# sen-ye/dmvae

Measured on AMD Instinct MI355X. Metric: images/sec DMVAE train step @256x256, higher is better.
Workload: dtype bf16

## Files before the change

### dmvae_amd/csrc/gemm_pp.hip

```cpp
#include "common.h"
#include "dmvae_hip.h"
#include <cstdlib>
#include <type_traits>

constexpr int GEMM_MAXBUF = 6;

namespace dmvae_gemm_pp {

struct Args {
  const bf16* x;
  const bf16* w;
  const void* bias;
  void* y;
  int M, N, K, lda, ldw, ldy;
  int act, bias_bf16;
  int H;
  unsigned wbytes;
  unsigned wsRow, wsK;
  int ntn, total;
  float inv_ntn;
  int tpb;
  float inv_tpb;
  unsigned sA, sB, sY, xbytes, ybytes;
  unsigned long long* dbg;
  int V, skS, T;
  float* slabs;
  unsigned* counters;
  unsigned slab_bytes;
  void* y2;
  int ldy2;
};

constexpr int SK_COHERENT = 1 | 16;
constexpr unsigned SENT = 0x80000000u;

__device__ __forceinline__ int swz64(int row) { return (0 - (row >> 2)) & 3; }

template <int N>
__device__ __forceinline__ void wait_vmcnt() {
  __builtin_amdgcn_s_waitcnt((N & 15) | 0x0F70 | ((N >> 4) << 14));
  asm volatile("" ::: "memory");
}

__device__ __forceinline__ float gelu_f(float x) { return dmvae_gelu_f(x); }

template <int TM, int TP, int WM, int WP, bool OUT_F32, int NBUF, bool BATCHED = false, bool SK = false>
__global__ __launch_bounds__(WM * WP * 64) void gemm_pp_kernel(Args a) {
#if __HIP_DEVICE_COMPILE__
  constexpr int PF = NBUF - 1;
  static_assert(!(SK && BATCHED) && !(SK && OUT_F32), "SK: single product, bf16 result");
  constexpr int CL = TM / WM / 16, BT = TP / WP / 16;
  constexpr int NW = WM * WP;
  static_assert(NW == 8 && CL * 16 * WM == TM && BT * 16 * WP == TP && CL * BT <= 32 && (CL == 4 || CL == 6 || CL == 8), "wave grid");
  constexpr int TILE_A = TM * 64, TILE_B = TP * 64, SLOT = TILE_A + TILE_B, RING = NBUF * SLOT;
  constexpr int NPA = (TM / 16 + NW - 1) / NW, NPB = (TP / 16 + NW - 1) / NW, NP = NPA + NPB;
  constexpr int CW = CL * 16;
  constexpr int BIAS_OFF = RING, DUMP_OFF = RING + 2048;
  constexpr int SPR = OUT_F32 ? (CL + 3) / 4 : 1;
  constexpr int NST = BT * 4 * SPR;
  extern __shared__ __attribute__((aligned(16))) char smem[];
  typedef unsigned u32x4 __attribute__((ext_vector_type(4)));
  typedef unsigned u32x3 __attribute__((ext_vector_type(3)));
  typedef unsigned u32x2 __attribute__((ext_vector_type(2)));

  const int tid = threadIdx.x, lane = tid & 63;
  const int wave = __builtin_amdgcn_readfirstlane(tid >> 6);
  const int grp = wave >> 2;
  const int wm = wave / WP, wp = wave % WP;
  const int nK = a.K >> 5;
  const unsigned bsz = a.bias_bf16 ? 2u : 4u;
  const bool gated = a.act == 6;
  const float inv_ntn = a.inv_ntn;

  const __amdgpu_buffer_rsrc_t rA = __builtin_amdgcn_make_buffer_rsrc((void*)a.w, 0, a.wbytes, 0x00020000);
  const __amdgpu_buffer_rsrc_t rB = __builtin_amdgcn_make_buffer_rsrc((void*)a.x, 0, BATCHED ? a.xbytes : (unsigned)a.M * (unsigned)a.lda * 2u, 0x00020000);
  const __amdgpu_buffer_rsrc_t rBias = __builtin_amdgcn_make_buffer_rsrc((void*)a.bias, 0, a.bias ? (unsigned)a.N * bsz : 0u, 0x00020000);
  const __amdgpu_buffer_rsrc_t rY = __builtin_amdgcn_make_buffer_rsrc(a.y, 0, BATCHED ? a.ybytes : (unsigned)a.M * (unsigned)a.ldy * (OUT_F32 ? 4u : 2u), 0x00020000);
  const __amdgpu_buffer_rsrc_t rY2 = __builtin_amdgcn_make_buffer_rsrc(a.y2, 0, a.y2 ? (unsigned)a.M * (unsigned)a.ldy2 * 2u : 0u, 0x00020000);

  auto calc = [&](unsigned work, unsigned (&vA)[NPA], unsigned (&vB)[NPB], unsigned& vBias, int& m0, int& n0, int& b0) {
    int lane_c = lane;
    asm volatile("" : "+v"(lane_c));
    const bool live = work < (unsigned)a.total;
    int wid = live ? (SK ? (int)work : (int)xcd_remap(work, a.total)) : 0;
    unsigned offA = 0, offB = 0;
    b0 = 0;
    if constexpr (BATCHED) {
      int b = (int)((float)wid * a.inv_tpb);
      int r = wid - b * a.tpb;
      if (r < 0) { b--; r += a.tpb; }
      if (r >= a.tpb) { b++; r -= a.tpb; }
      b0 = __builtin_amdgcn_readfirstlane(b);
      wid = r;
      offA = (unsigned)b0 * a.sA; offB = (unsigned)b0 * a.sB;
    }
    int mt = (int)((float)wid * inv_ntn);
    int nt = wid - mt * a.ntn;
    if (nt < 0) { mt--; nt += a.ntn; }
    if (nt >= a.ntn) { mt++; nt -= a.ntn; }
    m0 = __builtin_amdgcn_readfirstlane(mt) * TP;
    n0 = __builtin_amdgcn_readfirstlane(nt) * TM;
#pragma unroll
    for (int p = 0; p < NPA; p++) {
      const int rl = (wave * NPA + p) * 16 + (lane_c >> 2);
      const int wmr = rl / CW, r = rl % CW, i = r >> 4, c = r & 15;
      int n = n0 + wmr * CW + CL * c + i;
      bool n_ok = n < a.N;
      if (gated) {
        const int hid = (n0 >> 1) + wmr * (CW / 2) + (CL / 2) * c + (i % (CL / 2));
        n = (i < CL / 2 ? 0 : a.H) + hid;
        n_ok = hid < a.H;
      }
      const int ch = (lane_c & 3) ^ swz64(rl);
      vA[p] = (live && rl < TM && n_ok) ? (unsigned)n * a.wsRow + ch * 16u + offA : SENT;
    }
#pragma unroll
    for (int p = 0; p < NPB; p++) {
      const int rl = (wave * NPB + p) * 16 + (lane_c >> 2);
      const int m = m0 + rl;
      const int ch = (lane_c & 3) ^ swz64(rl);
      vB[p] = (live && rl < TP && m < a.M) ? (unsigned)m * (unsigned)a.lda * 2u + ch * 16u + offB : SENT;
    }
    const unsigned e0 = (unsigned)lane_c * (16u / bsz);
    if (gated) {
      const unsigned eh = e0 < (unsigned)(TM / 2) ? e0 : e0 - (unsigned)(TM / 2);
      const unsigned hid = (unsigned)(n0 >> 1) + eh;
      vBias = (live && wave == 0 && e0 < (unsigned)TM && hid < (unsigned)a.H) ? ((e0 < (unsigned)(TM / 2) ? 0u : (unsigned)a.H) + hid) * bsz : SENT;
    } else {
      vBias = (live && wave == 0 && e0 < (unsigned)TM && (unsigned)n0 + e0 < (unsigned)a.N) ? ((unsigned)n0 + e0) * bsz : SENT;
    }
  };
  auto issue_k = [&](const unsigned (&vA)[NPA], const unsigned (&vB)[NPB], unsigned kt, int slot) {
#pragma unroll
    for (int p = 0; p < NPA; p++) {
      const int g = wave * NPA + p;
      __builtin_amdgcn_raw_ptr_buffer_load_lds(rA, LPTR(smem + (g * 16 < TM ? slot + g * 1024 : DUMP_OFF)), 16, vA[p], kt * a.wsK, 0, 0);
    }
#pragma unroll
    for (int p = 0; p < NPB; p++) {
      const int g = wave * NPB + p;
      __builtin_amdgcn_raw_ptr_buffer_load_lds(rB, LPTR(smem + (g * 16 < TP ? slot + TILE_A + g * 1024 : DUMP_OFF)), 16, vB[p], kt * 64u, 0, 0);
    }
  };
  auto issue_bias = [&](unsigned vBias, int par) {
    __builtin_amdgcn_raw_ptr_buffer_load_lds(rBias, LPTR(smem + (wave == 0 ? BIAS_OFF + par * 1024 : DUMP_OFF)), 16, vBias, 0, 0, 0);
  };

  const int fr = (lane & 15) * 64 + (((lane >> 4) ^ swz64(lane & 15)) << 4);
  const int wbase = wm * (CW * 64) + fr;
  const int tbase = TILE_A + wp * (TP / WP) * 64 + fr;

  constexpr int MINSEG = 2 * PF + 2;
  struct Unit { int tile, kb, nk, p, P, i1; };
  auto bnd = [&](int v) -> int {
    if (a.skS > 0) {
      const int t = v / a.skS, p = v - t * a.skS;
      return t * nK + (p * nK) / a.skS;
    }
    int b = (int)((long long)v * (long long)a.T / (long long)a.V);
    const int r = b % nK;
    if (r < MINSEG) b -= r;
    else if (nK - r < MINSEG) b += nK - r;
    return b;
  };
  unsigned sk_work = blockIdx.x;
  int sk_pos = 0, sk_end = 0, sk_v = 0;
  bool sk_started = false;
  auto next_unit = [&]() -> Unit {
    Unit u = {a.total, 0, 2 * PF, 0, 1, 0};
    while (sk_pos >= sk_end) {
      if (sk_started) sk_work += gridDim.x;
      sk_started = true;
      if (sk_work >= (unsigned)a.V) return u;
      sk_v = (int)xcd_remap(sk_work, (unsigned)a.V);
      sk_pos = bnd(sk_v); sk_end = bnd(sk_v + 1);
    }
    const int tile = sk_pos / nK, lo = tile * nK, hi = lo + nK;
    u.tile = tile; u.kb = sk_pos - lo;
    const int ke = sk_end < hi ? sk_end - lo : nK;
    u.nk = ke - u.kb;
    sk_pos += u.nk;
    if (u.nk != nK) {
      int v = sk_v;
      while (v >= 1 && bnd(v) > lo) v--;
      u.i1 = v + 1;
      int w = sk_v + 1;
      while (w < a.V && bnd(w) < hi) w++;
      u.P = w - u.i1 + 1;
      u.p = u.kb == 0 ? 0 : sk_v - u.i1 + 1;
    }
    u.tile = __builtin_amdgcn_readfirstlane(u.tile); u.kb = __builtin_amdgcn_readfirstlane(u.kb); u.nk = __builtin_amdgcn_readfirstlane(u.nk);
    u.p = __builtin_amdgcn_readfirstlane(u.p); u.P = __builtin_amdgcn_readfirstlane(u.P); u.i1 = __builtin_amdgcn_readfirstlane(u.i1);
    return u;
  };
  Unit uc = {0, 0, nK, 0, 1, 0}, un = uc;

  f32x4 acc[CL][BT];
  bf16x8 wf[CL], tf[BT];
  unsigned vAc[NPA], vBc[NPB], vAn[NPA], vBn[NPB], vBiasN;
  int m0c, n0c, m0n = 0, n0n = 0, b0c = 0, b0n = 0;
  int slot_rd = 0, slot_wr = PF * SLOT, par = 0;
  int it = PF;


  auto kstep = [&](auto WAITc, auto MODEc) __attribute__((always_inline)) {
    constexpr int WAIT = decltype(WAITc)::value, MODE = decltype(MODEc)::value;
    const char* sw = smem + slot_rd + wbase;
    const char* st = smem + slot_rd + tbase;
#pragma unroll
    for (int j = 0; j < BT; j++) tf[j] = *reinterpret_cast<const bf16x8*>(st + j * 1024);
#pragma unroll
    for (int i = 0; i < CL; i++) wf[i] = *reinterpret_cast<const bf16x8*>(sw + i * 1024);
    if constexpr (MODE == 0) { issue_k(vAc, vBc, (unsigned)(it + (SK ? uc.kb : 0)), slot_wr); it++; }
    else {
      if constexpr (MODE == 1) issue_bias(vBiasN, par ^ 1);
      issue_k(vAn, vBn, (unsigned)(MODE - 1 + (SK ? un.kb : 0)), slot_wr);
    }
    slot_rd = slot_rd + SLOT == RING ? 0 : slot_rd + SLOT;
    slot_wr = slot_wr + SLOT == RING ? 0 : slot_wr + SLOT;
    if constexpr (WAIT >= 0) wait_vmcnt<WAIT>();
    __builtin_amdgcn_s_waitcnt(0xC07F);
    asm volatile("" ::: "memory");
    __builtin_amdgcn_sched_barrier(0);
    __builtin_amdgcn_s_barrier();
    __builtin_amdgcn_sched_barrier(0);
#pragma unroll
    for (int i = 0; i < CL; i++)
#pragma unroll
      for (int j = 0; j < BT; j++)
        asm volatile("v_mfma_f32_16x16x32_bf16 %0, %1, %2, %0" : "+a"(acc[i][j]) : "v"(tf[j]), "v"(wf[i]));
    __builtin_amdgcn_sched_barrier(0);
    __builtin_amdgcn_s_barrier();
    __builtin_amdgcn_sched_barrier(0);
  };
  using W_NO = std::integral_constant<int, -1>; using W_0 = std::integral_constant<int, 0>;
  using W_ST = std::integral_constant<int, (PF - 1) * NP>; using W_TL = std::integral_constant<int, (PF - 1) * NP + 1>;
  using M0_ = std::integral_constant<int, 0>;
  static_assert((PF - 1) * NP + 1 < 64, "vmcnt is a 6-bit counter");

  unsigned work = blockIdx.x;
  if constexpr (SK) { uc = next_unit(); work = (unsigned)uc.tile; }
  {
    unsigned vBiasC;
    calc(work, vAc, vBc, vBiasC, m0c, n0c, b0c);
    issue_bias(vBiasC, 0);
  }
#pragma unroll
  for (int u = 0; u < PF; u++) issue_k(vAc, vBc, (unsigned)(u + (SK ? uc.kb : 0)), u * SLOT);
  wait_vmcnt<0>();

  int tix = 0;
  auto stamp = [&](int k) { if (a.dbg && tid == 0 && tix < 4) a.dbg[((size_t)blockIdx.x * 4 + tix) * 8 + k] = __builtin_amdgcn_s_memtime(); };
  while (work < (unsigned)a.total) {
    stamp(0);
    __builtin_amdgcn_s_barrier();
    {
      const char* bl = smem + BIAS_OFF + par * 1024;
      int lane_b = lane;
      asm volatile("" : "+v"(lane_b));
      const int col = gated ? wm * (CW / 2) + (CL / 2) * (lane_b & 15) : wm * CW + CL * (lane_b & 15);
      const int hop = gated ? TM / 2 - CL / 2 : 0;
      float bv[8] = {0.f, 0.f, 0.f, 0.f, 0.f, 0.f, 0.f, 0.f};
      if (!a.bias || (SK && uc.p != 0)) {
      } else if (a.bias_bf16) {
#pragma unroll
        for (int h = 0; h < CL / 2; h++) {
          const bf16x2 b2 = *reinterpret_cast<const bf16x2*>(bl + (col + (h >= CL / 4 ? hop : 0)) * 2 + h * 4);
          bv[2 * h] = (float)b2[0]; bv[2 * h + 1] = (float)b2[1];
        }
      } else {
#pragma unroll
        for (int h = 0; h < CL / 2; h++) {
          const f32x2 b2 = *reinterpret_cast<const f32x2*>(bl + (col + (h >= CL / 4 ? hop : 0)) * 4 + h * 8);
          bv[2 * h] = b2[0]; bv[2 * h + 1] = b2[1];
        }
      }
#pragma unroll
      for (int i = 0; i < CL; i++)
#pragma unroll
        for (int j = 0; j < BT; j++) acc[i][j] = f32x4{bv[i], bv[i], bv[i], bv[i]};
    }
    stamp(1);
    unsigned next = work + gridDim.x;
    const int nkc = SK ? uc.nk : nK;
    if (grp == 1) __builtin_amdgcn_s_setprio(1);
    if (grp == 1) __builtin_amdgcn_s_barrier();
    it = PF;
    [&]<int... T>(std::integer_sequence<int, T...>) __attribute__((always_inline)) { (((void)T, kstep(W_NO{}, M0_{})), ...); }(std::make_integer_sequence<int, PF - 1>{});
    kstep(W_ST{}, M0_{});
#pragma unroll 1
    for (int t = PF; t < nkc - PF; t++) kstep(W_ST{}, M0_{});
    if constexpr (SK) { un = next_unit(); next = (unsigned)un.tile; }
    calc(next, vAn, vBn, vBiasN, m0n, n0n, b0n);
    [&]<int... J>(std::integer_sequence<int, J...>) __attribute__((always_inline)) { (kstep(W_TL{}, std::integral_constant<int, J + 1>{}), ...); }(std::make_integer_sequence<int, PF - 1>{});
    kstep(W_0{}, std::integral_constant<int, PF>{});
    if (grp == 0) __builtin_amdgcn_s_barrier();
    if (grp == 1) __builtin_amdgcn_s_setprio(0);
    asm volatile("s_nop 15\n\ts_nop 15" ::: "memory");
    stamp(2);

    bool sk_final = true;
    unsigned sk_base = 0;
    [[maybe_unused]] const __amdgpu_buffer_rsrc_t rS = __builtin_amdgcn_make_buffer_rsrc((void*)a.slabs, 0, SK ? a.slab_bytes : 0u, 0x00020000);
    constexpr unsigned SLOT_BYTES = (unsigned)TM * (unsigned)TP * 4u, WREG = (unsigned)CL * BT * 4u * 64u * 4u;
    if constexpr (SK) {
      if (uc.P > 1) {
        static_assert(!SK || CL % 4 == 0, "SK: 16-B pieces of a lane's columns");
        sk_base = (unsigned)wave * WREG;
        const unsigned own = (uc.p == 0 ? (unsigned)(a.V + uc.i1) : (unsigned)(uc.i1 + uc.p - 1)) * SLOT_BYTES + sk_base;
        int lane_s = lane;
        asm volatile("" : "+v"(lane_s));
        const unsigned vo = (unsigned)lane_s * 16u;
#pragma unroll
        for (int j = 0; j < BT; j++)
#pragma unroll
          for (int r = 0; r < 4; r++) {
            float v[8] = {0.f, 0.f, 0.f, 0.f, 0.f, 0.f, 0.f, 0.f};
#pragma unroll
            for (int i = 0; i < CL; i++) asm volatile("v_accvgpr_read_b32 %0, %1" : "=v"(v[i]) : "a"(acc[i][j][r]));
#pragma unroll
            for (int h = 0; h < CL / 4; h++) {
              const f32x4 o4 = {v[4 * h], v[4 * h + 1], v[4 * h + 2], v[4 * h + 3]};
              const u32x4 k4 = *reinterpret_cast<const u32x4*>(&o4);
              __builtin_amdgcn_raw_buffer_store_b128(k4, rS, vo, own + (unsigned)(((j * 4 + r) * (CL / 4) + h) * 1024), SK_COHERENT);
              asm volatile("s_nop 0" :: "v"(k4));
            }
          }
        stamp(4);
        wait_vmcnt<0>();
        stamp(5);
        unsigned old = 0;
        unsigned* cnt = a.counters + (size_t)uc.tile * 8 + wave;
        if (lane_s == 0) old = __hip_atomic_fetch_add(cnt, 1u, __ATOMIC_RELAXED, __HIP_MEMORY_SCOPE_AGENT);
        old = (unsigned)__builtin_amdgcn_readfirstlane((int)old);
        sk_final = old == (unsigned)(uc.P - 1);
        stamp(6);
        if (sk_final) {
          if (lane_s == 0) __hip_atomic_store(cnt, 0u, __ATOMIC_RELAXED, __HIP_MEMORY_SCOPE_AGENT);
        }
      }
    }

    if (sk_final) {
      int lane_o = lane;
      asm volatile("" : "+v"(lane_o));
      const int col = gated ? (n0c >> 1) + wm * (CW / 2) + (CL / 2) * (lane_o & 15) : n0c + wm * CW + CL * (lane_o & 15);
      const int row0 = m0c + wp * (TP / WP) + 4 * (lane_o >> 4);
      const unsigned ysoff = BATCHED ? (unsigned)b0c * a.sY : 0u;
      const bool c_ok = col < (gated ? a.H : a.N);
      auto body = [&](auto ACTc, auto SUMc) __attribute__((always_inline)) {
        constexpr int ACT = decltype(ACTc)::value;
        constexpr bool SUM = decltype(SUMc)::value;
#pragma unroll
        for (int j = 0; j < BT; j++) {
          [[maybe_unused]] float sm[4][8];
          if constexpr (SUM) {
#pragma unroll
            for (int r = 0; r < 4; r++)
#pragma unroll
              for (int i = 0; i < 8; i++) sm[r][i] = 0.f;
            const unsigned vo = (unsigned)lane_o * 16u;
#pragma unroll 1
            for (int q = 0; q < uc.P; q++) {
              if (q == uc.p) {
#pragma unroll
                for (int r = 0; r < 4; r++)
#pragma unroll
                  for (int i = 0; i < CL; i++) {
                    float t;
                    asm volatile("v_accvgpr_read_b32 %0, %1" : "=v"(t) : "a"(acc[i][j][r]));
                    sm[r][i] += t;
                  }
              } else {
                const unsigned src = (q == 0 ? (unsigned)(a.V + uc.i1) : (unsigned)(uc.i1 + q - 1)) * SLOT_BYTES + sk_base;
                u32x4 ld[4][CL / 4];
#pragma unroll
                for (int r = 0; r < 4; r++)
#pragma unroll
                  for (int h = 0; h < CL / 4; h++)
                    ld[r][h] = __builtin_amdgcn_raw_buffer_load_b128(rS, vo, src + (unsigned)(((j * 4 + r) * (CL / 4) + h) * 1024), SK_COHERENT);
#pragma unroll
                for (int r = 0; r < 4; r++)
#pragma unroll
                  for (int h = 0; h < CL / 4; h++) {
                    const f32x4 f = *reinterpret_cast<const f32x4*>(&ld[r][h]);
#pragma unroll
                    for (int e = 0; e < 4; e++) sm[r][4 * h + e] += f[e];
                  }
              }
            }
          }
#pragma unroll
          for (int r = 0; r < 4; r++) {
            float v[8] = {0.f, 0.f, 0.f, 0.f, 0.f, 0.f, 0.f, 0.f};
            if constexpr (SUM) {
#pragma unroll
              for (int i = 0; i < CL; i++) v[i] = sm[r][i];
            } else {
#pragma unroll
              for (int i = 0; i < CL; i++)
                asm volatile("v_accvgpr_read_b32 %0, %1" : "=v"(v[i]) : "a"(acc[i][j][r]));
            }
            if constexpr (ACT == 6) {
              if constexpr (!OUT_F32 && !BATCHED && (CL == 8 || CL == 4)) {
                if (a.y2) {
                  const int m2 = row0 + j * 16 + r;
                  const bool ok2 = c_ok && m2 < a.M;
                  const unsigned e1 = ((unsigned)m2 * (unsigned)a.ldy2 + (unsigned)col) * 2u, e2 = e1 + (unsigned)a.H * 2u;
                  if constexpr (CL == 8) {
                    const u32x2 p1 = {dmvae_pack_bf16x2(v[0], v[1]), dmvae_pack_bf16x2(v[2], v[3])}, p2 = {dmvae_pack_bf16x2(v[4], v[5]), dmvae_pack_bf16x2(v[6], v[7])};
                    __builtin_amdgcn_raw_buffer_store_b64(p1, rY2, ok2 ? e1 : SENT, 0, 0);
                    __builtin_amdgcn_raw_buffer_store_b64(p2, rY2, ok2 ? e2 : SENT, 0, 0);
                    asm volatile("s_nop 0" :: "v"(p1), "v"(p2));
                  } else {
                    const unsigned p1 = dmvae_pack_bf16x2(v[0], v[1]), p2 = dmvae_pack_bf16x2(v[2], v[3]);
                    __builtin_amdgcn_raw_buffer_store_b32(p1, rY2, ok2 ? e1 : SENT, 0, 0);
                    __builtin_amdgcn_raw_buffer_store_b32(p2, rY2, ok2 ? e2 : SENT, 0, 0);
                    asm volatile("s_nop 0" :: "v"(p1), "v"(p2));
                  }
                }
              }
#pragma unroll
              for (int i = 0; i < CL / 2; i++) {
                const float x1 = (float)(bf16)v[i], x2 = (float)(bf16)v[CL / 2 + i];
                v[i] = (float)(bf16)(x1 * sigmoidf_(x1)) * x2;
              }
            } else if constexpr (ACT != 0) {
#pragma unroll
              for (int i = 0; i < CL; i++) {
                const float x = (float)(bf16)v[i];
                v[i] = ACT == 5 ? gelu_f(x) : x * sigmoidf_(x);
              }
            }
            const int m = row0 + j * 16 + r;
            const bool ok = c_ok && m < a.M;
            const unsigned eo = (unsigned)m * (unsigned)a.ldy + (unsigned)col;
            if constexpr (ACT == 6) {
              if constexpr (CL == 8 && !OUT_F32) {
                const u32x2 o = {dmvae_pack_bf16x2(v[0], v[1]), dmvae_pack_bf16x2(v[2], v[3])};
                __builtin_amdgcn_raw_buffer_store_b64(o, rY, ok ? eo * 2u : SENT, ysoff, 0);
                asm volatile("s_nop 0" :: "v"(o));
              } else if constexpr (CL == 4 && !OUT_F32) {
                const unsigned o = dmvae_pack_bf16x2(v[0], v[1]);
                __builtin_amdgcn_raw_buffer_store_b32(o, rY, ok ? eo * 2u : SENT, ysoff, 0);
                asm volatile("s_nop 0" :: "v"(o));
              }
            } else if constexpr (OUT_F32 && CL == 6) {
#pragma unroll
              for (int e = 0; e < 3; e++) {
                const f32x2 o2 = {v[2 * e], v[2 * e + 1]};
                const u32x2 k2 = *reinterpret_cast<const u32x2*>(&o2);
                __builtin_amdgcn_raw_buffer_store_b64(k2, rY, (ok && col + 2 * e < a.N) ? eo * 4u + 8u * e : SENT, ysoff, 0);
                asm volatile("s_nop 0" :: "v"(k2));
              }
            } else if constexpr (OUT_F32) {
              const f32x4 o0 = {v[0], v[1], v[2], v[3]};
              const u32x4 k0 = *reinterpret_cast<const u32x4*>(&o0);
              __builtin_amdgcn_raw_buffer_store_b128(k0, rY, ok ? eo * 4u : SENT, ysoff, 0);
              if constexpr (CL == 8) {
                const f32x4 o1 = {v[4], v[5], v[6], v[7]};
                const u32x4 k1 = *reinterpret_cast<const u32x4*>(&o1);
                __builtin_amdgcn_raw_buffer_store_b128(k1, rY, ok ? eo * 4u + 16u : SENT, ysoff, 0);
                asm volatile("s_nop 0" :: "v"(k0), "v"(k1));
              } else {
                asm volatile("s_nop 0" :: "v"(k0));
              }
            } else if constexpr (CL == 8) {
              const u32x4 o = {dmvae_pack_bf16x2(v[0], v[1]), dmvae_pack_bf16x2(v[2], v[3]), dmvae_pack_bf16x2(v[4], v[5]), dmvae_pack_bf16x2(v[6], v[7])};
              __builtin_amdgcn_raw_buffer_store_b128(o, rY, ok ? eo * 2u : SENT, ysoff, 0);
              asm volatile("s_nop 0" :: "v"(o));
            } else if constexpr (CL == 6) {
              const u32x3 o = {dmvae_pack_bf16x2(v[0], v[1]), dmvae_pack_bf16x2(v[2], v[3]), dmvae_pack_bf16x2(v[4], v[5])};
              const bool full = col + 6 <= a.N;
              __builtin_amdgcn_raw_buffer_store_b96(o, rY, (ok && full) ? eo * 2u : SENT, ysoff, 0);
              if (__builtin_amdgcn_ballot_w64(ok && !full) != 0ull) {
#pragma unroll
                for (int e = 0; e < 2; e++)
                  __builtin_amdgcn_raw_buffer_store_b32(o[e], rY, (ok && !full && col + 2 * e < a.N) ? eo * 2u + 4u * e : SENT, ysoff, 0);
              }
              asm volatile("s_nop 0" :: "v"(o));
            } else {
              const u32x2 o = {dmvae_pack_bf16x2(v[0], v[1]), dmvae_pack_bf16x2(v[2], v[3])};
              __builtin_amdgcn_raw_buffer_store_b64(o, rY, ok ? eo * 2u : SENT, ysoff, 0);
              asm volatile("s_nop 0" :: "v"(o));
            }
          }
        }
      };
      auto by_act = [&](auto SUMc) __attribute__((always_inline)) {
        if (a.act == 0) body(std::integral_constant<int, 0>{}, SUMc);
        else if (a.act == 5) body(std::integral_constant<int, 5>{}, SUMc);
        else if (a.act == 6) body(std::integral_constant<int, 6>{}, SUMc);
        else body(std::integral_constant<int, 1>{}, SUMc);
      };
      if constexpr (SK) {
        if (uc.P > 1) by_act(std::true_type{});
        else by_act(std::false_type{});
      } else {
        by_act(std::false_type{});
      }
    }
    if (a.dbg) __builtin_amdgcn_s_barrier();
    stamp(3);
    tix++;
    work = next;
#pragma unroll
    for (int p = 0; p < NPA; p++) vAc[p] = vAn[p];
#pragma unroll
    for (int p = 0; p < NPB; p++) vBc[p] = vBn[p];
    m0c = m0n; n0c = n0n; b0c = b0n;
    if constexpr (SK) uc = un;
    par ^= 1;
  }
#endif
}

template <int TM, int TP, int WM, int WP, bool F32, bool BATCHED = false>
int launch(Args a, hipStream_t st, int batch = 1) {
  a.ntn = (a.N + TM - 1) / TM;
  a.tpb = ((a.M + TP - 1) / TP) * a.ntn;
  a.total = a.tpb * batch;
  DMVAE_CHECK_ARG(a.total > 0 && a.total < (1 << 24) && (long long)a.tpb * batch < (1 << 24),
                  "linear_bf16: %lld output tiles (the kernel's tile index arithmetic is exact below 2^24)", (long long)a.tpb * batch);
  a.inv_ntn = 1.0f / (float)a.ntn;
  a.inv_tpb = 1.0f / (float)a.tpb;
  const unsigned grid = a.total > 256 ? 256u : (unsigned)a.total;
  constexpr int slot = (TM + TP) * 64;
  constexpr int fit = (160 * 1024 - 3 * 1024) / slot;
  constexpr int nbuf = fit > GEMM_MAXBUF ? GEMM_MAXBUF : fit;
  static_assert(nbuf >= 4, "LDS");
  constexpr int lds = nbuf * slot + 3 * 1024;
  static bool attr_done = false;
  if (!attr_done) {
    (void)hipFuncSetAttribute(reinterpret_cast<const void*>(gemm_pp_kernel<TM, TP, WM, WP, F32, nbuf, BATCHED>), hipFuncAttributeMaxDynamicSharedMemorySize, lds);
    attr_done = true;
  }
  hipLaunchKernelGGL((gemm_pp_kernel<TM, TP, WM, WP, F32, nbuf, BATCHED>), dim3(grid), dim3(WM * WP * 64), lds, st, a);
  DMVAE_CHECK_LAUNCH();
  return 0;
}
constexpr int SK_GRID = 256, SK_MAX_TILES = 2048, SK_COUNTER_BYTES = SK_MAX_TILES * 8 * 4;
struct SkTile { int tm, tp, minseg; };
static inline SkTile sk_tile(int tile) { return tile == 1 ? SkTile{256, 128, 12} : SkTile{256, 256, 8}; }
template <int TM, int TP, int WM, int WP>
static int launch_sk_t(Args a, int splits, hipStream_t st) {
  a.ntn = (a.N + TM - 1) / TM;
  a.tpb = ((a.M + TP - 1) / TP) * a.ntn;
  a.total = a.tpb;
  a.inv_ntn = 1.0f / (float)a.ntn;
  a.inv_tpb = 1.0f / (float)a.tpb;
  a.skS = splits;
  a.V = splits > 0 ? a.total * splits : SK_GRID;
  a.T = a.total * (a.K >> 5);
  const unsigned grid = a.V > SK_GRID ? (unsigned)SK_GRID : (unsigned)a.V;
  constexpr int slot = (TM + TP) * 64;
  constexpr int fit = (160 * 1024 - 3 * 1024) / slot;
  constexpr int nbuf = fit > GEMM_MAXBUF ? GEMM_MAXBUF : fit;
  constexpr int lds = nbuf * slot + 3 * 1024;
  static bool attr_done = false;
  if (!attr_done) {
    (void)hipFuncSetAttribute(reinterpret_cast<const void*>(gemm_pp_kernel<TM, TP, WM, WP, false, nbuf, false, true>), hipFuncAttributeMaxDynamicSharedMemorySize, lds);
    attr_done = true;
  }
  hipLaunchKernelGGL((gemm_pp_kernel<TM, TP, WM, WP, false, nbuf, false, true>), dim3(grid), dim3(512), lds, st, a);
  DMVAE_CHECK_LAUNCH();
  return 0;
}
static int launch_sk(Args a, int splits, int tile, hipStream_t st) {
  return tile == 1 ? launch_sk_t<256, 128, 4, 2>(a, splits, st) : launch_sk_t<256, 256, 2, 4>(a, splits, st);
}
static bool sk_ok(int M, int N, int K, int splits, int tile) {
  if (!(M >= 64 && N > 0 && N % 8 == 0 && K % 32 == 0 && K >= 384 && splits >= 0 && splits <= 8 && (tile == 0 || tile == 1))) return false;
  const SkTile t = sk_tile(tile);
  const long long tiles = (long long)((M + t.tp - 1) / t.tp) * ((N + t.tm - 1) / t.tm);
  const int nK = K >> 5;
  if (tiles > SK_MAX_TILES || tiles * nK >= (1ll << 30)) return false;
  if (splits == 0) return tiles * nK / SK_GRID >= 2 * t.minseg && nK >= 2 * t.minseg;
  return nK / splits >= t.minseg && tiles * splits <= 4096;
}

struct Cfg { int tm, tp; float cost; };
static const Cfg g_cfg[] = {
    {256, 256, 1.00f}, {256, 224, 0.94f}, {256, 192, 0.885f}, {256, 160, 0.80f}, {256, 128, 0.67f},
    {128, 448, 1.02f}, {128, 384, 0.93f}, {128, 256, 0.70f},  {192, 256, 0.90f}, {192, 320, 1.12f},
    {192, 128, 0.54f}, {128, 192, 0.54f},
};
constexpr int NCFG = sizeof(g_cfg) / sizeof(g_cfg[0]);

static int g_forced = -1;
static int plan(int M, int N, int K, bool gated = false) {
  const int forced = g_forced;
  if (forced >= 0 && forced < NCFG && !(gated && g_cfg[forced].tm == 192)) return forced;
  (void)K;
  constexpr int NPLAN = 10;
  int best = 0;
  float best_t = 1e30f;
  for (int c = 0; c < NPLAN; c++) {
    if (gated && g_cfg[c].tm == 192) continue;
    const long long tiles = (long long)((M + g_cfg[c].tp - 1) / g_cfg[c].tp) * ((N + g_cfg[c].tm - 1) / g_cfg[c].tm);
    const float frac = (float)tiles / 256.0f, whole = 0.85f * (float)((tiles + 255) / 256);
    const float t = (frac > whole ? frac : whole) * g_cfg[c].cost;
    if (t < best_t * 0.999f) { best_t = t; best = c; }
  }
  return best;
}

template <bool F32>
static int dispatch(int cfg, const Args& a, hipStream_t st) {
  switch (cfg) {
    case 0: return launch<256, 256, 2, 4, F32>(a, st);
    case 1: return launch<256, 224, 4, 2, F32>(a, st);
    case 2: return launch<256, 192, 2, 4, F32>(a, st);
    case 3: return launch<256, 160, 4, 2, F32>(a, st);
    case 4: return launch<256, 128, 4, 2, F32>(a, st);
    case 5: return launch<128, 448, 2, 4, F32>(a, st);
    case 6: return launch<128, 384, 2, 4, F32>(a, st);
    case 7: return launch<128, 256, 2, 4, F32>(a, st);
    case 8: return launch<192, 256, 2, 4, F32>(a, st);
    case 9: return launch<192, 320, 2, 4, F32>(a, st);
    case 10: return launch<192, 128, 2, 4, F32>(a, st);
    default: return launch<128, 192, 2, 4, F32>(a, st);
  }
}

}

static unsigned long long* g_gemm_dbg = nullptr;
extern "C" void dmvae_debug_gemm_timing(void* buf) { g_gemm_dbg = (unsigned long long*)buf; }
extern "C" void dmvae_debug_gemm_cfg(int cfg) { dmvae_gemm_pp::g_forced = cfg; }

extern "C" int dmvae_linear_bf16_plan(int M, int N, int K, int* tile_cols, int* tile_rows) {
  using namespace dmvae_gemm_pp;
  const int c = plan(M, N, K);
  if (tile_cols) *tile_cols = g_cfg[c].tm;
  if (tile_rows) *tile_rows = g_cfg[c].tp;
  return c;
}

extern "C" int dmvae_linear_bf16_batched_supported(int batch, int M, int N, int K) {
  return (batch > 0 && M >= 64 && N > 0 && N % 8 == 0 && K >= 384 && K % 32 == 0) ? 1 : 0;
}
extern "C" int dmvae_linear_bf16_batched(const void* x, const void* w, void* y, int batch, int M, int N, int K, int lda, int ldw, int ldy, long long sx, long long sw,
                                         long long sy, int out_f32, hipStream_t stream) {
  using namespace dmvae_gemm_pp;
  DMVAE_CHECK_ARG(x && w && y, "linear_bf16_batched: null operand");
  DMVAE_CHECK_ARG(dmvae_linear_bf16_batched_supported(batch, M, N, K), "linear_bf16_batched: need K %% 32 == 0, K >= 384, N %% 8 == 0, M >= 64 (batch %d, M %d, N %d, K %d)",
                  batch, M, N, K);
  DMVAE_CHECK_ARG(lda >= K && ldw >= K && ldy >= N && lda % 8 == 0 && ldw % 8 == 0 && ldy % 8 == 0, "linear_bf16_batched: leading dimensions must cover the rows and be multiples of 8");
  DMVAE_CHECK_ARG(sx >= (long long)M * lda && sw >= (long long)N * ldw && sy >= (long long)M * ldy && sx % 8 == 0 && sw % 8 == 0 && sy % 8 == 0,
                  "linear_bf16_batched: batch strides must cover one product's operand and be multiples of 8 elements");
  const long long xb = ((long long)(batch - 1) * sx + (long long)M * lda) * 2, wb = ((long long)(batch - 1) * sw + (long long)N * ldw) * 2;
  const long long yb = ((long long)(batch - 1) * sy + (long long)M * ldy) * (out_f32 ? 4 : 2);
  DMVAE_CHECK_ARG(xb < (1ll << 31) && wb < (1ll << 31) && yb < (1ll << 31), "linear_bf16_batched: operands are addressed through 32-bit buffer offsets (2 GiB each over the whole batch)");
  Args a;
  a.x = (const bf16*)x; a.w = (const bf16*)w; a.bias = nullptr; a.y = y;
  a.M = M; a.N = N; a.K = K; a.lda = lda; a.ldw = ldw; a.ldy = ldy;
  a.act = 0; a.bias_bf16 = 0; a.H = N / 2; a.ntn = 0; a.total = 0; a.inv_ntn = 0.f; a.dbg = nullptr;
  a.V = a.skS = a.T = 0; a.slabs = nullptr; a.counters = nullptr; a.slab_bytes = 0u; a.y2 = nullptr; a.ldy2 = 0;
  a.wbytes = (unsigned)wb; a.xbytes = (unsigned)xb; a.ybytes = (unsigned)yb;
  a.wsRow = (unsigned)ldw * 2u; a.wsK = 64u;
  a.sA = (unsigned)(sw * 2); a.sB = (unsigned)(sx * 2); a.sY = (unsigned)(sy * (out_f32 ? 4 : 2));
  static const int cand[3] = {0, 4, 7};
  int best = 0;
  float best_t = 1e30f;
  for (int i = 0; i < 3; i++) {
    const Cfg& c = g_cfg[cand[i]];
    const long long tiles = (long long)batch * ((M + c.tp - 1) / c.tp) * ((N + c.tm - 1) / c.tm);
    const float frac = (float)tiles / 256.0f, whole = 0.85f * (float)((tiles + 255) / 256);
    const float t = (frac > whole ? frac : whole) * c.cost;
    if (t < best_t * 0.999f) { best_t = t; best = cand[i]; }
  }
  if (out_f32) {
    if (best == 0) return launch<256, 256, 2, 4, true, true>(a, stream, batch);
    if (best == 4) return launch<256, 128, 4, 2, true, true>(a, stream, batch);
    return launch<128, 256, 2, 4, true, true>(a, stream, batch);
  }
  if (best == 0) return launch<256, 256, 2, 4, false, true>(a, stream, batch);
  if (best == 4) return launch<256, 128, 4, 2, false, true>(a, stream, batch);
  return launch<128, 256, 2, 4, false, true>(a, stream, batch);
}

extern "C" int dmvae_linear_bf16_sk_supported(int M, int N, int K, int splits, int tile) { return dmvae_gemm_pp::sk_ok(M, N, K, splits, tile) ? 1 : 0; }
extern "C" size_t dmvae_linear_bf16_sk_workspace(int M, int N, int K, int splits, int tile) {
  using namespace dmvae_gemm_pp;
  if (!sk_ok(M, N, K, splits, tile)) return 0;
  const SkTile t = sk_tile(tile);
  const long long tiles = (long long)((M + t.tp - 1) / t.tp) * ((N + t.tm - 1) / t.tm);
  const long long V = splits > 0 ? tiles * splits : SK_GRID;
  return (size_t)SK_COUNTER_BYTES + (size_t)(2 * V) * t.tm * t.tp * 4;
}
extern "C" int dmvae_linear_bf16_sk(const void* x, const void* w, const void* bias, void* y, void* workspace, size_t workspace_bytes, int splits, int tile, int M, int N,
                                    int K, int lda, int ldw, int ldy, int act, int bias_bf16, int w_layout, hipStream_t stream) {
  using namespace dmvae_gemm_pp;
  DMVAE_CHECK_ARG(x && w && y && workspace, "linear_bf16_sk: null operand");
  DMVAE_CHECK_ARG(sk_ok(M, N, K, splits, tile), "linear_bf16_sk: M %d N %d K %d splits %d tile %d not taken (dmvae_linear_bf16_sk_supported)", M, N, K, splits, tile);
  DMVAE_CHECK_ARG(w_layout == 0 || w_layout == 1, "linear_bf16_sk: w_layout must be 0 (row-major [N][ldw]) or 1 (K-tile-major [K / 32][N][32])");
  DMVAE_CHECK_ARG(lda >= K && (w_layout == 1 || ldw >= K) && ldy >= (act == 6 ? N / 2 : N) && lda % 8 == 0 && ldw % 8 == 0 && ldy % 8 == 0,
                  "linear_bf16_sk: leading dimensions must cover the rows and be multiples of 8");
  DMVAE_CHECK_ARG(act == 0 || act == 1 || act == 5 || act == 6, "linear_bf16_sk: act must be 0 (none), 1 (SiLU), 5 (GELU) or 6 (SwiGLU over the [x1 | x2] halves of N)");
  DMVAE_CHECK_ARG(act != 6 || N % 16 == 0, "linear_bf16_sk: the SwiGLU epilogue needs N %% 16 == 0");
  const long long wb = w_layout == 1 ? (long long)N * K * 2 : (long long)N * ldw * 2;
  DMVAE_CHECK_ARG((long long)M * lda * 2 < (1ll << 31) && wb < (1ll << 31) && (long long)M * ldy * 2 < (1ll << 31),
                  "linear_bf16_sk: operands are addressed through 32-bit buffer offsets (2 GiB each)");
  const size_t need = dmvae_linear_bf16_sk_workspace(M, N, K, splits, tile);
  DMVAE_CHECK_ARG(workspace_bytes >= need && need - SK_COUNTER_BYTES < (1ull << 32), "linear_bf16_sk: workspace too small (need %zu bytes, see dmvae_linear_bf16_sk_workspace)", need);
  Args a;
  a.x = (const bf16*)x; a.w = (const bf16*)w; a.bias = bias; a.y = y;
  a.M = M; a.N = N; a.K = K; a.lda = lda; a.ldw = ldw; a.ldy = ldy;
  a.act = act; a.bias_bf16 = bias_bf16; a.H = N / 2; a.ntn = 0; a.total = 0; a.inv_ntn = 0.f; a.dbg = g_gemm_dbg;
  a.wbytes = (unsigned)wb; a.tpb = 0; a.inv_tpb = 0.f; a.sA = a.sB = a.sY = a.xbytes = a.ybytes = 0u;
  a.wsRow = w_layout == 1 ? 64u : (unsigned)ldw * 2u;
  a.wsK = w_layout == 1 ? (unsigned)N * 64u : 64u;
  a.y2 = nullptr; a.ldy2 = 0;
  a.counters = (unsigned*)workspace;
  a.slabs = (float*)((char*)workspace + SK_COUNTER_BYTES);
  a.slab_bytes = (unsigned)(need - SK_COUNTER_BYTES);
  return launch_sk(a, splits, tile, stream);
}

static int linear_bf16_impl(const void* x, const void* w, const void* bias, void* y, void* y2, int ldy2, int M, int N, int K, int lda, int ldw, int ldy,
                            int act, int bias_bf16, int out_f32, int w_layout, hipStream_t stream);
extern "C" int dmvae_linear_bf16(const void* x, const void* w, const void* bias, void* y, int M, int N, int K, int lda, int ldw, int ldy,
                                 int act, int bias_bf16, int out_f32, int w_layout, hipStream_t stream) {
  return linear_bf16_impl(x, w, bias, y, nullptr, 0, M, N, K, lda, ldw, ldy, act, bias_bf16, out_f32, w_layout, stream);
}
extern "C" int dmvae_linear_bf16_swiglu_pre(const void* x, const void* w, const void* bias, void* g, void* x12, int M, int N, int K, int lda, int ldw, int ldg,
                                            int ldx12, int bias_bf16, int w_layout, hipStream_t stream) {
  DMVAE_CHECK_ARG(x12 && ldx12 >= N && ldx12 % 8 == 0, "linear_bf16_swiglu_pre: x12 must be given with ldx12 >= N, a multiple of 8");
  return linear_bf16_impl(x, w, bias, g, x12, ldx12, M, N, K, lda, ldw, ldg, 6, bias_bf16, 0, w_layout, stream);
}
static int linear_bf16_impl(const void* x, const void* w, const void* bias, void* y, void* y2, int ldy2, int M, int N, int K, int lda, int ldw, int ldy,
                            int act, int bias_bf16, int out_f32, int w_layout, hipStream_t stream) {
  using namespace dmvae_gemm_pp;
  DMVAE_CHECK_ARG(x && w && y, "linear_bf16: null operand");
  DMVAE_CHECK_ARG(M > 0 && N > 0 && K >= 384 && K % 32 == 0 && N % 8 == 0, "linear_bf16: need K %% 32 == 0, K >= 384 and N %% 8 == 0 (M %d, N %d, K %d)", M, N, K);
  DMVAE_CHECK_ARG(w_layout == 0 || w_layout == 1, "linear_bf16: w_layout must be 0 (row-major [N][ldw]) or 1 (K-tile-major [K / 32][N][32])");
  DMVAE_CHECK_ARG(lda >= K && (w_layout == 1 || ldw >= K) && ldy >= (act == 6 ? N / 2 : N) && lda % 8 == 0 && ldw % 8 == 0 && ldy % 8 == 0,
                  "linear_bf16: leading dimensions must cover the rows and be multiples of 8");
  DMVAE_CHECK_ARG(act == 0 || act == 1 || act == 5 || act == 6, "linear_bf16: act must be 0 (none), 1 (SiLU), 5 (GELU) or 6 (SwiGLU over the [x1 | x2] halves of N)");
  DMVAE_CHECK_ARG(act != 6 || (!out_f32 && N % 16 == 0), "linear_bf16: the SwiGLU epilogue writes bf16 and needs N %% 16 == 0");
  const long long wb = w_layout == 1 ? (long long)N * K * 2 : (long long)N * ldw * 2;
  DMVAE_CHECK_ARG((long long)M * lda * 2 < (1ll << 31) && wb < (1ll << 31) && (long long)M * ldy * (out_f32 ? 4 : 2) < (1ll << 31),
                  "linear_bf16: operands are addressed through 32-bit buffer offsets (2 GiB each)");
  Args a;
  a.x = (const bf16*)x; a.w = (const bf16*)w; a.bias = bias; a.y = y;
  a.M = M; a.N = N; a.K = K; a.lda = lda; a.ldw = ldw; a.ldy = ldy;
  a.act = act; a.bias_bf16 = bias_bf16; a.H = N / 2; a.ntn = 0; a.total = 0; a.inv_ntn = 0.f; a.dbg = g_gemm_dbg;
  a.V = a.skS = a.T = 0; a.slabs = nullptr; a.counters = nullptr; a.slab_bytes = 0u; a.y2 = y2; a.ldy2 = ldy2;
  DMVAE_CHECK_ARG(!y2 || (long long)M * ldy2 * 2 < (1ll << 31), "linear_bf16_swiglu_pre: x12 is addressed through 32-bit buffer offsets (2 GiB)");
  a.wbytes = (unsigned)wb; a.tpb = 0; a.inv_tpb = 0.f; a.sA = a.sB = a.sY = a.xbytes = a.ybytes = 0u;
  a.wsRow = w_layout == 1 ? 64u : (unsigned)ldw * 2u;
  a.wsK = w_layout == 1 ? (unsigned)N * 64u : 64u;
  const int cfg = plan(M, N, K, act == 6);
  return out_f32 ? dispatch<true>(cfg, a, stream) : dispatch<false>(cfg, a, stream);
}
```

Baseline: 496.7.

## Skip MFMAs on ragged last row-tile and model partial tiles in planner

For output tiles where fewer than TP rows remain, the B-row mapping is remapped so valid rows are packed into the first accumulator blocks of each wave. Each wave then skips the MFMA groups and stores for blocks beyond its valid count via a scalar branch inside the asm. The XCD remap now applies only to full tiles, so ragged tiles run as trailing work. The tile planner gains a cost model that charges partial tiles at reduced cost, which may pick different configs. This adds a scalar compare and branch per MFMA group and more complex indexing, with correctness risk in the remapped epilogue row math.

```diff
diff --git a/dmvae_amd/csrc/gemm_pp.hip b/dmvae_amd/csrc/gemm_pp.hip
--- a/dmvae_amd/csrc/gemm_pp.hip
+++ b/dmvae_amd/csrc/gemm_pp.hip
@@ -18,6 +18,7 @@
   unsigned wbytes;
   unsigned wsRow, wsK;
   int ntn, total;
+  int full;
   float inv_ntn;
   int tpb;
   float inv_tpb;
@@ -82,7 +83,7 @@
     int lane_c = lane;
     asm volatile("" : "+v"(lane_c));
     const bool live = work < (unsigned)a.total;
-    int wid = live ? (SK ? (int)work : (int)xcd_remap(work, a.total)) : 0;
+    int wid = live ? (SK ? (int)work : BATCHED ? (int)xcd_remap(work, a.total) : work < (unsigned)a.full ? (int)xcd_remap(work, a.full) : (int)work) : 0;
     unsigned offA = 0, offB = 0;
     b0 = 0;
     if constexpr (BATCHED) {
@@ -116,8 +117,9 @@
     }
 #pragma unroll
     for (int p = 0; p < NPB; p++) {
-      const int rl = (wave * NPB + p) * 16 + (lane_c >> 2);
-      const int m = m0 + rl;
+      const int g = wave * NPB + p;
+      const int rl = g * 16 + (lane_c >> 2);
+      const int m = m0 + (a.M - m0 < TP ? ((g % BT) * WP + g / BT) * 16 + (lane_c >> 2) : rl);
       const int ch = (lane_c & 3) ^ swz64(rl);
       vB[p] = (live && rl < TP && m < a.M) ? (unsigned)m * (unsigned)a.lda * 2u + ch * 16u + offB : SENT;
     }
@@ -172,7 +174,8 @@
       if (sk_started) sk_work += gridDim.x;
       sk_started = true;
       if (sk_work >= (unsigned)a.V) return u;
-      sk_v = (int)xcd_remap(sk_work, (unsigned)a.V);
+      const unsigned vfull = a.skS > 0 ? (unsigned)(a.full * a.skS) : (unsigned)a.V;
+      sk_v = sk_work < vfull ? (int)xcd_remap(sk_work, vfull) : (int)sk_work;
       sk_pos = bnd(sk_v); sk_end = bnd(sk_v + 1);
     }
     const int tile = sk_pos / nK, lo = tile * nK, hi = lo + nK;
@@ -203,6 +206,7 @@
   int it = PF;
 
 
+  int nvb = BT;
   auto kstep = [&](auto WAITc, auto MODEc) __attribute__((always_inline)) {
     constexpr int WAIT = decltype(WAITc)::value, MODE = decltype(MODEc)::value;
     const char* sw = smem + slot_rd + wbase;
@@ -224,11 +228,26 @@
     __builtin_amdgcn_sched_barrier(0);
     __builtin_amdgcn_s_barrier();
     __builtin_amdgcn_sched_barrier(0);
-#pragma unroll
-    for (int i = 0; i < CL; i++)
-#pragma unroll
-      for (int j = 0; j < BT; j++)
-        asm volatile("v_mfma_f32_16x16x32_bf16 %0, %1, %2, %0" : "+a"(acc[i][j]) : "v"(tf[j]), "v"(wf[i]));
+#define DMVAE_MFMA_(n) "v_mfma_f32_16x16x32_bf16 %" #n ", %[t], %[w" #n "], %" #n "\n\t"
+#define DMVAE_SKIP_ "s_cmp_le_i32 %[nv], %[jj]\n\ts_cbranch_scc1 .Lgemm_pp_skip%=\n\t"
+#pragma unroll
+    for (int j = 0; j < BT; j++) {
+      if constexpr (CL == 4)
+        asm volatile(DMVAE_SKIP_ DMVAE_MFMA_(0) DMVAE_MFMA_(1) DMVAE_MFMA_(2) DMVAE_MFMA_(3) ".Lgemm_pp_skip%=:"
+                     : "+a"(acc[0][j]), "+a"(acc[1][j]), "+a"(acc[2][j]), "+a"(acc[3][j])
+                     : [t] "v"(tf[j]), [w0] "v"(wf[0]), [w1] "v"(wf[1]), [w2] "v"(wf[2]), [w3] "v"(wf[3]), [nv] "s"(nvb), [jj] "s"(j) : "scc");
+      else if constexpr (CL == 6)
+        asm volatile(DMVAE_SKIP_ DMVAE_MFMA_(0) DMVAE_MFMA_(1) DMVAE_MFMA_(2) DMVAE_MFMA_(3) DMVAE_MFMA_(4) DMVAE_MFMA_(5) ".Lgemm_pp_skip%=:"
+                     : "+a"(acc[0][j]), "+a"(acc[1][j]), "+a"(acc[2][j]), "+a"(acc[3][j]), "+a"(acc[4][j]), "+a"(acc[5][j])
+                     : [t] "v"(tf[j]), [w0] "v"(wf[0]), [w1] "v"(wf[1]), [w2] "v"(wf[2]), [w3] "v"(wf[3]), [w4] "v"(wf[4]), [w5] "v"(wf[5]), [nv] "s"(nvb), [jj] "s"(j) : "scc");
+      else
+        asm volatile(DMVAE_SKIP_ DMVAE_MFMA_(0) DMVAE_MFMA_(1) DMVAE_MFMA_(2) DMVAE_MFMA_(3) DMVAE_MFMA_(4) DMVAE_MFMA_(5) DMVAE_MFMA_(6) DMVAE_MFMA_(7) ".Lgemm_pp_skip%=:"
+                     : "+a"(acc[0][j]), "+a"(acc[1][j]), "+a"(acc[2][j]), "+a"(acc[3][j]), "+a"(acc[4][j]), "+a"(acc[5][j]), "+a"(acc[6][j]), "+a"(acc[7][j])
+                     : [t] "v"(tf[j]), [w0] "v"(wf[0]), [w1] "v"(wf[1]), [w2] "v"(wf[2]), [w3] "v"(wf[3]), [w4] "v"(wf[4]), [w5] "v"(wf[5]), [w6] "v"(wf[6]), [w7] "v"(wf[7]),
+                       [nv] "s"(nvb), [jj] "s"(j) : "scc");
+    }
+#undef DMVAE_MFMA_
+#undef DMVAE_SKIP_
     __builtin_amdgcn_sched_barrier(0);
     __builtin_amdgcn_s_barrier();
     __builtin_amdgcn_sched_barrier(0);
@@ -253,6 +272,9 @@
   auto stamp = [&](int k) { if (a.dbg && tid == 0 && tix < 4) a.dbg[((size_t)blockIdx.x * 4 + tix) * 8 + k] = __builtin_amdgcn_s_memtime(); };
   while (work < (unsigned)a.total) {
     stamp(0);
+    const int rows_left = a.M - m0c;
+    const bool rag = rows_left < TP;
+    nvb = rag ? __builtin_amdgcn_readfirstlane((((rows_left + 15) >> 4) - wp + WP - 1) / WP) : BT;
     __builtin_amdgcn_s_barrier();
     {
       const char* bl = smem + BIAS_OFF + par * 1024;
@@ -312,7 +334,8 @@
         asm volatile("" : "+v"(lane_s));
         const unsigned vo = (unsigned)lane_s * 16u;
 #pragma unroll
-        for (int j = 0; j < BT; j++)
+        for (int j = 0; j < BT; j++) {
+          const unsigned voj = j < nvb ? vo : SENT;
 #pragma unroll
           for (int r = 0; r < 4; r++) {
             float v[8] = {0.f, 0.f, 0.f, 0.f, 0.f, 0.f, 0.f, 0.f};
@@ -322,10 +345,11 @@
             for (int h = 0; h < CL / 4; h++) {
               const f32x4 o4 = {v[4 * h], v[4 * h + 1], v[4 * h + 2], v[4 * h + 3]};
               const u32x4 k4 = *reinterpret_cast<const u32x4*>(&o4);
-              __builtin_amdgcn_raw_buffer_store_b128(k4, rS, vo, own + (unsigned)(((j * 4 + r) * (CL / 4) + h) * 1024), SK_COHERENT);
+              __builtin_amdgcn_raw_buffer_store_b128(k4, rS, voj, own + (unsigned)(((j * 4 + r) * (CL / 4) + h) * 1024), SK_COHERENT);
               asm volatile("s_nop 0" :: "v"(k4));
             }
           }
+        }
         stamp(4);
         wait_vmcnt<0>();
         stamp(5);
@@ -345,7 +369,8 @@
       int lane_o = lane;
       asm volatile("" : "+v"(lane_o));
       const int col = gated ? (n0c >> 1) + wm * (CW / 2) + (CL / 2) * (lane_o & 15) : n0c + wm * CW + CL * (lane_o & 15);
-      const int row0 = m0c + wp * (TP / WP) + 4 * (lane_o >> 4);
+      const int row0 = m0c + wp * (rag ? 16 : TP / WP) + 4 * (lane_o >> 4);
+      const int jrows = rag ? 16 * WP : 16;
       const unsigned ysoff = BATCHED ? (unsigned)b0c * a.sY : 0u;
       const bool c_ok = col < (gated ? a.H : a.N);
       auto body = [&](auto ACTc, auto SUMc) __attribute__((always_inline)) {
@@ -359,7 +384,7 @@
             for (int r = 0; r < 4; r++)
 #pragma unroll
               for (int i = 0; i < 8; i++) sm[r][i] = 0.f;
-            const unsigned vo = (unsigned)lane_o * 16u;
+            const unsigned vo = j < nvb ? (unsigned)lane_o * 16u : SENT;
 #pragma unroll 1
             for (int q = 0; q < uc.P; q++) {
               if (q == uc.p) {
@@ -404,7 +429,7 @@
             if constexpr (ACT == 6) {
               if constexpr (!OUT_F32 && !BATCHED && (CL == 8 || CL == 4)) {
                 if (a.y2) {
-                  const int m2 = row0 + j * 16 + r;
+                  const int m2 = row0 + j * jrows + r;
                   const bool ok2 = c_ok && m2 < a.M;
                   const unsigned e1 = ((unsigned)m2 * (unsigned)a.ldy2 + (unsigned)col) * 2u, e2 = e1 + (unsigned)a.H * 2u;
                   if constexpr (CL == 8) {
@@ -432,7 +457,7 @@
                 v[i] = ACT == 5 ? gelu_f(x) : x * sigmoidf_(x);
               }
             }
-            const int m = row0 + j * 16 + r;
+            const int m = row0 + j * jrows + r;
             const bool ok = c_ok && m < a.M;
             const unsigned eo = (unsigned)m * (unsigned)a.ldy + (unsigned)col;
             if constexpr (ACT == 6) {
@@ -520,6 +545,7 @@
   a.ntn = (a.N + TM - 1) / TM;
   a.tpb = ((a.M + TP - 1) / TP) * a.ntn;
   a.total = a.tpb * batch;
+  a.full = (a.M / TP) * a.ntn;
   DMVAE_CHECK_ARG(a.total > 0 && a.total < (1 << 24) && (long long)a.tpb * batch < (1 << 24),
                   "linear_bf16: %lld output tiles (the kernel's tile index arithmetic is exact below 2^24)", (long long)a.tpb * batch);
   a.inv_ntn = 1.0f / (float)a.ntn;
@@ -547,6 +573,7 @@
   a.ntn = (a.N + TM - 1) / TM;
   a.tpb = ((a.M + TP - 1) / TP) * a.ntn;
   a.total = a.tpb;
+  a.full = (a.M / TP) * a.ntn;
   a.inv_ntn = 1.0f / (float)a.ntn;
   a.inv_tpb = 1.0f / (float)a.tpb;
   a.skS = splits;
@@ -579,15 +606,32 @@
   return nK / splits >= t.minseg && tiles * splits <= 4096;
 }
 
-struct Cfg { int tm, tp; float cost; };
+struct Cfg { int tm, tp; float cost; int wp; };
 static const Cfg g_cfg[] = {
-    {256, 256, 1.00f}, {256, 224, 0.94f}, {256, 192, 0.885f}, {256, 160, 0.80f}, {256, 128, 0.67f},
-    {128, 448, 1.02f}, {128, 384, 0.93f}, {128, 256, 0.70f},  {192, 256, 0.90f}, {192, 320, 1.12f},
-    {192, 128, 0.54f}, {128, 192, 0.54f},
+    {256, 256, 1.00f, 4}, {256, 224, 0.94f, 2}, {256, 192, 0.885f, 4}, {256, 160, 0.80f, 2}, {256, 128, 0.67f, 2},
+    {128, 448, 1.02f, 4}, {128, 384, 0.93f, 4}, {128, 256, 0.70f, 4},  {192, 256, 0.90f, 4}, {192, 320, 1.12f, 4},
+    {192, 128, 0.54f, 4}, {128, 192, 0.54f, 4},
 };
 constexpr int NCFG = sizeof(g_cfg) / sizeof(g_cfg[0]);
 
 static int g_forced = -1;
+constexpr float RAG_FLOOR = 0.45f;
+static float plan_time(const Cfg& c, int M, int N) {
+  const long long ntn = (N + c.tm - 1) / c.tm, full = (long long)(M / c.tp) * ntn;
+  const int rem = M % c.tp;
+  float r = 0.f;
+  if (rem) {
+    const int vb = (rem + 15) / 16, bt = c.tp / 16 / c.wp;
+    const float fl = RAG_FLOOR / c.cost;
+    r = (float)((vb + c.wp - 1) / c.wp) / (float)bt;
+    if (r < fl) r = fl;
+    if (r > 1.f || full == 0) r = 1.f;
+  }
+  const long long slack = (256 - full % 256) % 256;
+  const bool beside = !rem || ntn <= slack;
+  const float frac = ((float)full + (beside ? (float)ntn * r : 0.f)) / 256.0f, whole = 0.85f * (float)((full + 255) / 256);
+  return ((frac > whole ? frac : whole) + (beside ? 0.f : r)) * c.cost;
+}
 static int plan(int M, int N, int K, bool gated = false) {
   const int forced = g_forced;
   if (forced >= 0 && forced < NCFG && !(gated && g_cfg[forced].tm == 192)) return forced;
@@ -597,9 +641,7 @@
   float best_t = 1e30f;
   for (int c = 0; c < NPLAN; c++) {
     if (gated && g_cfg[c].tm == 192) continue;
-    const long long tiles = (long long)((M + g_cfg[c].tp - 1) / g_cfg[c].tp) * ((N + g_cfg[c].tm - 1) / g_cfg[c].tm);
-    const float frac = (float)tiles / 256.0f, whole = 0.85f * (float)((tiles + 255) / 256);
-    const float t = (frac > whole ? frac : whole) * g_cfg[c].cost;
+    const float t = plan_time(g_cfg[c], M, N);
     if (t < best_t * 0.999f) { best_t = t; best = c; }
   }
   return best;
```

After: 496.4 (median of 2 runs). Within noise of the previous version (-0.1%).
